# VUmcCGP/wisecondor

Hardware: AMD Instinct MI355X
Metric: newref bin-pair distances/sec (higher is better)
Workload: dtype f64; 1 GPU; cfg2: newref 100 samples x 250 kb bins (11087 masked bins, refsize 100); parallelism=newref sharded by single rank, symmetric tiles, 1 rank(s), world_size=1

## Files before the change

### wisecondor_amd/csrc/newref.hip

```cpp
#include <cstring>
#include "ctx.h"

#include <algorithm>
#include <stdlib.h>

namespace {

constexpr int TB = 128;
constexpr int BK = 32;
constexpr int LDA = 36;
constexpr int LDT = 68;
constexpr int ROLE_ROWS = 1;
constexpr int ROLE_COLS = 2;
constexpr int MAX_SAMPLE_COLS = 4096;
constexpr int LIST_CAP = 1024;
constexpr int K_MAX = 1024;
constexpr int GL_ROW = 16;
constexpr int GL_STAGE = 2 * TB * GL_ROW;
#define WC_ADMIT_ALL FLT_MAX
constexpr double SENTINEL_DISTANCE = 1e10;

typedef float f32x16 __attribute__((ext_vector_type(16)));
typedef float f32x4 __attribute__((ext_vector_type(4)));
typedef _Float16 f16x8 __attribute__((ext_vector_type(8)));
// ... 772 lines not shown
            for (int o = 32; o > 0; o >>= 1) my = fmax(my, __shfl_xor(my, o));
            if (lane == 0) red[tid >> 6] = my;
            wc_sync();
            U = red[0];
            for (int q = 1; q < NT / 64; ++q) U = fmax(U, red[q]);
            if (!(U == U) || (!admit_all && !(U <= (double)thr_f))) fallback = true;
        }
        {
            const float bad = *a.bad_norm;
            if (bad < INFINITY) {
                const double ni = sqrt(fmax((double)a.norm_lo[row] + (double)nhi_f, 0.0));
                if (!((sqrt(fmax(U, 0.0)) + ni) * (1.0 + 1e-3) < (double)bad * (1.0 - 1e-3))) fallback = true;
            }
        }
        if (!fallback) {
            for (int t0 = 0; t0 < n; t0 += NT) {
                int t = t0 + tid;
                bool keep = false;
                int j = 0;
                if (t < n) {
                    j = (int)(uint32_t)ent[t];
                    keep = (double)wc::f32_from_ordered((uint32_t)(ent[t] >> 32)) <= U;
                }
                unsigned long long m = __ballot(keep);
                int base = 0;
                if (lane == 0 && m) base = atomicAdd(&s_tmp[2], __popcll(m));
                base = __shfl(base, 0);
                int at = base + __popcll(m & ((1ull << lane) - 1ull));
                if (keep && at < RMAX) cj[at] = j;
            }
            wc_sync();
            R = s_tmp[2];
            if (R > RMAX) fallback = true;
        }
    }
    if (fallback) {
        if (tid == 0) {
            int at = atomicAdd(a.fb_count, 1);
            a.fb_rows[at] = (int)row;
            a.row_stat[row] = -1;
        }
        return;
    }

    {
        constexpr bool seq = SEQ;
        const int l8 = tid & 7, r0 = tid >> 3;
        for (int b0 = 0; b0 < R; b0 += CB) {
            const int nb = (R - b0) < CB ? (R - b0) : CB;
            unsigned int src[NP];
            f64x2 pre[NP];
            auto fetch = [&](unsigned int so) {
                if ((int64_t)so + ST_CH <= a.S) {
#pragma unroll
                    for (int p = 0; p < NP; ++p) pre[p] = *(const f64x2_u *)&a.X[src[p] + so];
                } else {
                    const int64_t s0 = (int64_t)so + 2 * l8;
#pragma unroll
                    for (int p = 0; p < NP; ++p) {
                        pre[p].x = s0 < a.S ? a.X[src[p] + so] : 0.0;
                        pre[p].y = s0 + 1 < a.S ? a.X[src[p] + so + 1] : 0.0;
                    }
                }
            };
#pragma unroll
            for (int p = 0; p < NP; ++p) {
                int rr = r0 + RP * p;
                src[p] = (unsigned int)cj[b0 + (rr < nb ? rr : 0)] * (unsigned int)a.S + 2u * (unsigned int)l8;
            }
            fetch(0u);
            double acc = 0.0;
            double r[8] = {0, 0, 0, 0, 0, 0, 0, 0};
            double vs[10] = {0, 0, 0, 0, 0, 0, 0, 0, 0, 0};
            int sp = 0, leaf = 0;
            bool in_tail = false;
            int2 lf = seq ? make_int2(0, 0) : a.pw_prog[0];
            for (int64_t c0 = 0; c0 < a.S; c0 += ST_CH) {
                wc_sync();
                {
                    f64x2 x2;
                    if (c0 + ST_CH <= a.S && a.xs_in_lds) {
                        x2 = *(const f64x2 *)&xi[c0 + 2 * l8];
                    } else {
                        const int64_t s0 = c0 + 2 * l8;
                        x2.x = s0 < a.S ? xi[s0] : 0.0;
                        x2.y = s0 + 1 < a.S ? xi[s0 + 1] : 0.0;
                    }
#pragma unroll
                    for (int p = 0; p < NP; ++p) {
                        const double d0 = pre[p].x - x2.x, d1 = pre[p].y - x2.y;
                        f64x2 sq2;
                        sq2.x = d0 * d0;
                        sq2.y = d1 * d1;
                        *(f64x2 *)&stage[(r0 + RP * p) * ST_LD + 2 * l8] = sq2;
                    }
                }
                wc_sync();
                if (c0 + ST_CH < a.S) fetch((unsigned int)(c0 + ST_CH));
                if (SEQ && tid < CB && c0 + ST_CH <= a.S && a.xs_in_lds) {
                    const double *sp_ = &stage[tid * ST_LD];
#pragma unroll
                    for (int e = 0; e < ST_CH; e += 2) {
                        const f64x2 v = *(const f64x2 *)(sp_ + e);
                        acc = acc + v.x;
                        acc = acc + v.y;
                    }
                } else if (tid < CB) {
                    const bool full = c0 + ST_CH <= a.S && a.xs_in_lds;
#pragma unroll
                    for (int g = 0; g < 2; ++g) {
                        const int64_t base = c0 + 8 * g;
                        if (base >= a.S) break;
                        const int cntg = (a.S - base) < 8 ? (int)(a.S - base) : 8;
                        double sq[8];
                        if (full) {
                            const double *sp_ = &stage[tid * ST_LD + 8 * g];
#pragma unroll
                            for (int e = 0; e < 8; e += 2) {
                                const f64x2 v = *(const f64x2 *)(sp_ + e);
                                sq[e] = v.x;
                                sq[e + 1] = v.y;
                            }
                        } else {
#pragma unroll
                            for (int e = 0; e < 8; ++e) sq[e] = (e < cntg) ? stage[tid * ST_LD + 8 * g + e] : 0.0;
                        }
                        if (seq || in_tail || cntg < 8) {
                            for (int e = 0; e < cntg; ++e) acc = acc + sq[e];
                        } else {
#pragma unroll
                            for (int e = 0; e < 8; ++e) r[e] = r[e] + sq[e];
                            if (base + 8 == (int64_t)(lf.x - (lf.x & 7))) {
                                double val = ((r[0] + r[1]) + (r[2] + r[3])) + ((r[4] + r[5]) + (r[6] + r[7]));
#pragma unroll
                                for (int e = 0; e < 8; ++e) r[e] = 0.0;
                                if (lf.x & 7) {
                                    acc = val;
                                    in_tail = true;
                                } else {
                                    wc::stack_set(vs, sp++, val);
                                    for (int q = 0; q < lf.y; ++q) {
                                        double right = wc::stack_get(vs, --sp), left = wc::stack_get(vs, sp - 1);
                                        wc::stack_set(vs, sp - 1, left + right);
                                    }
                                    ++leaf;
                                    if (leaf < a.pw_leaves) lf = a.pw_prog[leaf];
                                }
                            }
                        }
                    }
                }
            }
            if (!seq) {
                if (in_tail) {
                    wc::stack_set(vs, sp++, acc);
                    for (int q = 0; q < lf.y; ++q) {
                        double right = wc::stack_get(vs, --sp), left = wc::stack_get(vs, sp - 1);
                        wc::stack_set(vs, sp - 1, left + right);
                    }
                }
                acc = vs[0];
            }
            if (tid < nb) {
                bool ok = acc < SENTINEL_DISTANCE;
                dk[b0 + tid] = ok ? wc::f64_ordered(acc) : ~0ull;
                jv[b0 + tid] = ok ? cj[b0 + tid] : 0x40000000 + b0 + tid;
            }
        }
    }
    const int64_t cs = a.chrom_off[ch], ce = a.chrom_off[ch + 1];
    const int64_t orow = row - a.row_begin;
    wc_sync();
    {
        if (tid == 0 && (R & 1)) { dk[R] = ~0ull; jv[R] = 0x7FFFFFFF; }
        wc_sync();
        for (int t = tid; t < R; t += NT) {
            const unsigned long long mine = dk[t];
            const int myj = jv[t];
            int rank = 0;
            for (int u = 0; u < R; u += 2) {
                const u64x2 kk = *(const u64x2 *)&dk[u];
                const int2 jj = *(const int2 *)&jv[u];
                rank += (kk.x < mine) | ((kk.x == mine) & (jj.x < myj));
                rank += (kk.y < mine) | ((kk.y == mine) & (jj.y < myj));
            }
            if (rank < a.k) {
                int32_t oi = -1;
                double od = SENTINEL_DISTANCE;
                if (mine != ~0ull) {
                    oi = (int32_t)(myj < cs ? myj : myj - (ce - cs));
                    od = wc::f64_from_ordered(mine);
                }
                a.idx_out[orow * a.k + rank] = oi;
                a.dist_out[orow * a.k + rank] = od;
            }
        }
        for (int t = R + tid; t < a.k; t += NT) {
            a.idx_out[orow * a.k + t] = -1;
            a.dist_out[orow * a.k + t] = SENTINEL_DISTANCE;
        }
    }
    if (tid == 0) a.row_stat[row] = R;
}

constexpr int PS_MAX = 512;

struct PickArgs {
    FinishArgs f;
    int *pairs;
    int ps;
};

template <int NE, bool LEAN>
__device__ inline int pick_row(const PickArgs &p, int64_t row, int lane, int n, bool admit_all, float thr_f,
                               float nhi_f, const unsigned long long (&spec)[8]) {
    const FinishArgs &a = p.f;
    const unsigned long long *lst = a.list + row * a.cap;
    unsigned long long ent[LEAN ? 1 : NE];
    float nh[LEAN ? 1 : NE];
    uint32_t key[LEAN ? NE : 1];
    if constexpr (LEAN) {
#pragma unroll
        for (int e = 0; e < NE; ++e) {
            const int t = e * 64 + lane;
            key[e] = t < n ? (uint32_t)((e < 8 ? spec[e] : lst[t]) >> 32) : 0xFFFFFFFFu;
        }
    } else {
#pragma unroll
        for (int e = 0; e < NE; ++e) {
            const int t = e * 64 + lane;
            ent[e] = t < n ? (e < 8 ? spec[e] : lst[t]) : ~0ull;
        }
#pragma unroll
        for (int e = 0; e < NE; ++e) {
            const int t = e * 64 + lane;
            nh[e] = t < n ? a.norm_hi[(int)(uint32_t)ent[e]] : 0.f;
        }
    }
    auto KU = [&](int e) -> uint32_t { if constexpr (LEAN) return key[e]; else return (uint32_t)(ent[e] >> 32); };
    auto IDX = [&](int e) -> uint32_t { if constexpr (LEAN) return (uint32_t)lst[e * 64 + lane]; else return (uint32_t)ent[e]; };
    double U = INFINITY;
    if (n < a.k) {
        if (!admit_all) return -1;
    } else {
        uint32_t kmin = 0xFFFFFFFFu, kmax = 0u;
#pragma unroll
        for (int e = 0; e < NE; ++e)
            if (e * 64 + lane < n) {
                const uint32_t ku = KU(e);
                kmin = ku < kmin ? ku : kmin;
                kmax = ku > kmax ? ku : kmax;
            }
        for (int o = 32; o > 0; o >>= 1) {
            const uint32_t a2 = (uint32_t)__shfl_xor((int)kmin, o), b2 = (uint32_t)__shfl_xor((int)kmax, o);
            kmin = a2 < kmin ? a2 : kmin;
            kmax = b2 > kmax ? b2 : kmax;
        }
        long long lo = (long long)kmin - 1, hi = (long long)kmax;
        uint32_t res = kmax;
        while (hi - lo > 4096) {
            const uint32_t trial = (uint32_t)(lo + ((hi - lo) >> 1));
            int c = 0;
#pragma unroll
            for (int e = 0; e < NE; ++e) c += __popcll(__ballot(KU(e) <= trial));
            if (c >= a.k) { hi = (long long)trial; res = trial; if (c == a.k) break; }
            else lo = (long long)trial;
        }
        const double nhi = (double)nhi_f;
        double my = -INFINITY;
#pragma unroll
        for (int e = 0; e < NE; ++e) {
            const uint32_t ku = KU(e);
            if (e * 64 + lane < n && ku <= res) {
                float slack;
                if constexpr (LEAN) slack = a.norm_hi[(int)IDX(e)]; else slack = nh[e];
                const double ub = (double)wc::f32_from_ordered(ku) + (nhi + (double)slack) + 1e-36;
                my = fmax(my, ub);
            }
        }
        for (int o = 32; o > 0; o >>= 1) my = fmax(my, __shfl_xor(my, o));
        U = my;
        if (!(U == U) || (!admit_all && !(U <= (double)thr_f))) return -1;
    }
    {
        const float bad = *a.bad_norm;
        if (bad < INFINITY) {
            const double ni = sqrt(fmax((double)a.norm_lo[row] + (double)nhi_f, 0.0));
            if (!((sqrt(fmax(U, 0.0)) + ni) * (1.0 + 1e-3) < (double)bad * (1.0 - 1e-3))) return -1;
        }
    }
    int base = 0;
    int *out = p.pairs + row * RMAX;
#pragma unroll
    for (int e = 0; e < NE; ++e) {
        const bool keep = e * 64 + lane < n && (double)wc::f32_from_ordered(KU(e)) <= U;
        const unsigned long long m = __ballot(keep);
        const int at = base + __popcll(m & ((1ull << lane) - 1ull));
        if (keep && at < RMAX) out[at] = (int)IDX(e);
        base += __popcll(m);
    }
    return base;
}

__global__ __launch_bounds__(256, 7) void k_pick(PickArgs p) {
    const FinishArgs &a = p.f;
    const int lane = threadIdx.x & 63;
    const int64_t row = a.row_begin + (int64_t)blockIdx.x * 4 + (threadIdx.x >> 6);
    if (row >= a.row_end) return;
    unsigned long long spec[8];
#pragma unroll
    for (int e = 0; e < 8; ++e) spec[e] = a.list[row * a.cap + e * 64 + lane];
    const int c = a.cnt[row];
    const float thr_f = a.thr[row];
    const float nhi_f = a.norm_hi[row];
    const int ch = a.chrom_of_row[row];
    const bool admit_all = (thr_f == WC_ADMIT_ALL);
    const bool exact = c > a.cap || ((a.lone_mask >> ch) & 1ull);
    int R = -1;
    if (!exact) R = c <= 512 ? pick_row<8, false>(p, row, lane, c, admit_all, thr_f, nhi_f, spec)
                             : pick_row<LIST_CAP / 64, true>(p, row, lane, c, admit_all, thr_f, nhi_f, spec);
    if (lane != 0) return;
    if (R < 0 || R > RMAX) {
        const int at = atomicAdd(a.fb_count, 1);
        a.fb_rows[at] = (int)row;
        a.row_stat[row] = -1;
        return;
    }
    a.row_stat[row] = R;
}

__device__ inline void vs_set(double (&v)[8], int i, double x) {
    switch (i) {
        case 0: v[0] = x; break; case 1: v[1] = x; break; case 2: v[2] = x; break; case 3: v[3] = x; break;
        case 4: v[4] = x; break; case 5: v[5] = x; break; case 6: v[6] = x; break; default: v[7] = x; break;
    }
}
__device__ inline double vs_get(const double (&v)[8], int i) {
    switch (i) {
        case 0: return v[0]; case 1: return v[1]; case 2: return v[2]; case 3: return v[3];
        case 4: return v[4]; case 5: return v[5]; case 6: return v[6]; default: return v[7];
    }
}

template <bool SEQ>
struct RowSum {
    double acc;
    double r[8];
    double vs[8];
    int sp, leaf;
    bool in_tail;
    int2 lf;
    __device__ inline void init(const FinishArgs &a) {
        acc = 0.0;
#pragma unroll
        for (int e = 0; e < 8; ++e) r[e] = 0.0;
#pragma unroll
        for (int e = 0; e < 8; ++e) vs[e] = 0.0;
        sp = 0; leaf = 0; in_tail = false;
        lf = SEQ ? make_int2(0, 0) : a.pw_prog[0];
    }
    __device__ inline void chunk_regs(const FinishArgs &a, const double (&v)[ST_CH], int64_t c0, bool full) {
        if (SEQ) {
#pragma unroll
            for (int e = 0; e < ST_CH; ++e) acc = acc + v[e];
            return;
        }
#pragma unroll
        for (int g = 0; g < 2; ++g) {
            const int64_t base = c0 + 8 * g;
            if (base >= a.S) break;
            const int cntg = full ? 8 : ((a.S - base) < 8 ? (int)(a.S - base) : 8);
            if (in_tail || cntg < 8) {
#pragma unroll
                for (int e = 0; e < 8; ++e)
                    if (e < cntg) acc = acc + v[8 * g + e];
            } else {
#pragma unroll
                for (int e = 0; e < 8; ++e) r[e] = r[e] + v[8 * g + e];
                leaf_end(a, base);
            }
        }
    }
    __device__ inline void group_regs(const FinishArgs &a, const double (&v)[8], int64_t base, int cntg) {
        if (in_tail || cntg < 8) {
#pragma unroll
            for (int e = 0; e < 8; ++e)
                if (e < cntg) acc = acc + v[e];
        } else {
#pragma unroll
            for (int e = 0; e < 8; ++e) r[e] = r[e] + v[e];
            leaf_end(a, base);
        }
    }
    __device__ inline void leaf_end(const FinishArgs &a, int64_t base) {
        if (base + 8 == (int64_t)(lf.x - (lf.x & 7))) {
            const double val = ((r[0] + r[1]) + (r[2] + r[3])) + ((r[4] + r[5]) + (r[6] + r[7]));
#pragma unroll
            for (int e = 0; e < 8; ++e) r[e] = 0.0;
            if (lf.x & 7) {
                acc = val;
                in_tail = true;
            } else {
                vs_set(vs, sp++, val);
                for (int q = 0; q < lf.y; ++q) {
                    const double right = vs_get(vs, --sp), left = vs_get(vs, sp - 1);
                    vs_set(vs, sp - 1, left + right);
                }
                ++leaf;
                if (leaf < a.pw_leaves) lf = a.pw_prog[leaf];
            }
        }
    }
    __device__ inline double result() {
        if (SEQ) return acc;
        if (in_tail) {
            vs_set(vs, sp++, acc);
            for (int q = 0; q < lf.y; ++q) {
                const double right = vs_get(vs, --sp), left = vs_get(vs, sp - 1);
                vs_set(vs, sp - 1, left + right);
            }
        }
        return vs[0];
    }
};

__device__ inline void wave_lds_fence() {
    __builtin_amdgcn_fence(__ATOMIC_RELEASE, "wavefront");
    __builtin_amdgcn_wave_barrier();
    __builtin_amdgcn_fence(__ATOMIC_ACQUIRE, "wavefront");
}

constexpr int SLAB_DOUBLES = 64 * ST_CH;
template <bool SEQ, bool GLDS>
__global__ __launch_bounds__(PS_MAX, (SEQ && !GLDS) ? 4 : (SEQ ? 5 : 3)) void k_rescore(PickArgs p, const double *__restrict__ Xp, int Sp) {
    const FinishArgs &a = p.f;
    extern __shared__ __attribute__((aligned(16))) double rs_dyn[];
    const int tid = threadIdx.x, lane = tid & 63, w = __builtin_amdgcn_readfirstlane(tid >> 6);
    const int64_t row = a.row_begin + blockIdx.x;
    const int cj_first = p.pairs[row * RMAX + tid];
    const int R = a.row_stat[row];
    double *xs = rs_dyn;
    char *slab = reinterpret_cast<char *>(rs_dyn + Sp + w * SLAB_DOUBLES);
    {
        const double *xi = Xp + row * Sp;
        for (int s = tid; s < Sp; s += p.ps) xs[s] = xi[s];
    }
    if (R < 0) return;
    wc_sync();
    const int l8 = lane & 7, r0 = lane >> 3;
    constexpr int NP = 8;
    constexpr int TRIPS = RMAX / 128;
    auto swz = [](int r) { return ((r >> 1) & 3) | (((r >> 4) & 1) << 2); };
    int waddr[NP], raddr[NP];
#pragma unroll
    for (int q = 0; q < NP; ++q) {
        const int rw = r0 + 8 * q;
        waddr[q] = rw * 128 + ((l8 ^ swz(rw)) << 4);
        raddr[q] = lane * 128 + ((q ^ swz(lane)) << 4);
    }
    unsigned long long my_d[TRIPS];
    int my_j[TRIPS];
    int trip = 0;
    const int nchunk = Sp / ST_CH;
    const char *base = reinterpret_cast<const char *>(Xp);
    for (int b0 = w * 64; b0 < R; b0 += p.ps, ++trip) {
        const int nb = R - b0 < 64 ? R - b0 : 64;
        const int *cjp = p.pairs + row * RMAX + b0;
        int cj = trip == 0 ? cj_first : cjp[lane < nb ? lane : 0];
        if (trip == 0) cj = __shfl(cj, lane < nb ? lane : 0);
        unsigned int src[NP];
        RowSum<SEQ> sum;
        sum.init(a);
        if constexpr (GLDS) {
            const int l4 = lane & 3, rq = lane >> 2;
#pragma unroll
            for (int j = 0; j < 4; ++j) {
                const int rw = 16 * j + rq;
                src[j] = ((unsigned int)__shfl(cj, rw) * (unsigned int)Sp + 2u * (unsigned int)(l4 ^ ((rw >> 2) & 3))) * 8u;
            }
            int rd[4];
#pragma unroll
            for (int q = 0; q < 4; ++q) rd[q] = lane * 64 + ((q ^ ((lane >> 2) & 3)) << 4);
            auto dma = [&](int c, int half) {
                const char *cb = base + (size_t)c * (ST_CH * 8) + half * 64;
                char *dst = slab + half * 4096;
#pragma unroll
                for (int j = 0; j < 4; ++j)
                    __builtin_amdgcn_global_load_lds((glb_void_t *)(cb + src[j]), (lds_void_t *)(dst + j * 1024), 16, 0, 0);
            };
            dma(0, 0);
            dma(0, 1);
            for (int c = 0; c < nchunk; ++c) {
                __builtin_amdgcn_s_waitcnt(0x0070);
                __builtin_amdgcn_wave_barrier();
                f64x2 t[8];
#pragma unroll
                for (int q = 0; q < 4; ++q) t[q] = *(const f64x2 *)(slab + rd[q]);
#pragma unroll
                for (int q = 0; q < 4; ++q) t[4 + q] = *(const f64x2 *)(slab + 4096 + rd[q]);
                __builtin_amdgcn_s_waitcnt(0xC07F);
                __builtin_amdgcn_wave_barrier();
                if (c + 1 < nchunk) { dma(c + 1, 0); dma(c + 1, 1); }
                double v[ST_CH];
#pragma unroll
                for (int q = 0; q < NP; ++q) {
                    const f64x2 x2 = *(const f64x2 *)&xs[c * ST_CH + 2 * q];
                    const double d0 = t[q].x - x2.x, d1 = t[q].y - x2.y;
                    v[2 * q] = d0 * d0;
                    v[2 * q + 1] = d1 * d1;
                }
                sum.chunk_regs(a, v, (int64_t)c * ST_CH, (c + 1) * ST_CH <= a.S);
            }
        } else {
#pragma unroll
        for (int q = 0; q < NP; ++q)
            src[q] = ((unsigned int)__shfl(cj, r0 + 8 * q) * (unsigned int)Sp + 2u * (unsigned int)l8) * 8u;
        f64x2 pre[NP];
#pragma unroll
        for (int q = 0; q < NP; ++q) pre[q] = *(const f64x2 *)(base + src[q]);
        for (int c = 0; c < nchunk; ++c) {
            const f64x2 x2 = *(const f64x2 *)&xs[c * ST_CH + 2 * l8];
            wave_lds_fence();
#pragma unroll
            for (int q = 0; q < NP; ++q) {
                const double d0 = pre[q].x - x2.x, d1 = pre[q].y - x2.y;
                f64x2 sq2;
                sq2.x = d0 * d0;
                sq2.y = d1 * d1;
                *(f64x2 *)(slab + waddr[q]) = sq2;
            }
            wave_lds_fence();
            if (c + 1 < nchunk) {
                const char *cb = base + (size_t)(c + 1) * (ST_CH * 8);
#pragma unroll
                for (int q = 0; q < NP; ++q) pre[q] = *(const f64x2 *)(cb + src[q]);
            }
            double v[ST_CH];
#pragma unroll
            for (int q = 0; q < NP; ++q) {
                const f64x2 t2 = *(const f64x2 *)(slab + raddr[q]);
                v[2 * q] = t2.x;
                v[2 * q + 1] = t2.y;
            }
            sum.chunk_regs(a, v, (int64_t)c * ST_CH, (c + 1) * ST_CH <= a.S);
        }
        }
        const double d = sum.result();
        const bool ok = lane < nb && d < SENTINEL_DISTANCE;
        const unsigned long long dd = ok ? wc::f64_ordered(d) : ~0ull;
        const int jj = ok ? cj : 0x40000000 + b0 + lane;
#pragma unroll
        for (int t = 0; t < TRIPS; ++t)
            if (t == trip) { my_d[t] = dd; my_j[t] = jj; }
    }
    wc_sync();
    unsigned long long *dk = reinterpret_cast<unsigned long long *>(rs_dyn + Sp);
    unsigned long long *sd = dk + RMAX + 2;
    int *jv = reinterpret_cast<int *>(sd + RMAX);
    int *sj = jv + RMAX + 2;
    {
        int t2 = 0;
        for (int b0 = w * 64; b0 < R; b0 += p.ps, ++t2) {
#pragma unroll
            for (int t = 0; t < TRIPS; ++t)
                if (t == t2 && b0 + lane < R) { dk[b0 + lane] = my_d[t]; jv[b0 + lane] = my_j[t]; }
        }
    }
    if (tid == 0 && (R & 1)) dk[R] = ~0ull;
    for (int t = tid; t < R; t += p.ps) sj[t] = -1;
    wc_sync();
    for (int t = tid; t < R; t += p.ps) {
        const unsigned long long mine = dk[t];
        int rank = 0;
        for (int u = 0; u < R; u += 2) {
            const u64x2 kk = *(const u64x2 *)&dk[u];
            rank += kk.x < mine;
            rank += kk.y < mine;
        }
        sd[rank] = mine;
        sj[rank] = jv[t];
    }
    wc_sync();
    int hole = 0;
    for (int t = tid; t < R; t += p.ps) hole |= sj[t] == -1;
    if (wc_sync_or(hole)) {
        for (int t = tid; t < R; t += p.ps) {
            const unsigned long long mine = dk[t];
            const int myj = jv[t];
            int rank = 0;
            for (int u = 0; u < R; ++u) rank += (dk[u] < mine) | ((dk[u] == mine) & (jv[u] < myj));
            sd[rank] = mine;
            sj[rank] = myj;
        }
        wc_sync();
    }
    const int ch = a.chrom_of_row[row];
    const int64_t cs = a.chrom_off[ch], ce = a.chrom_off[ch + 1];
    const int64_t orow = row - a.row_begin;
    for (int t = tid; t < a.k; t += p.ps) {
        int32_t oi = -1;
        double od = SENTINEL_DISTANCE;
        if (t < R && sd[t] != ~0ull) {
            const int myj = sj[t];
            oi = (int32_t)(myj < cs ? myj : myj - (ce - cs));
            od = wc::f64_from_ordered(sd[t]);
        }
        a.idx_out[orow * a.k + t] = oi;
        a.dist_out[orow * a.k + t] = od;
    }
}

template <bool SEQ>
__device__ inline void fb_fill_order(const FinishArgs &a, int64_t row, const double *xi, int64_t j0, int64_t j1,
                                     unsigned long long *__restrict__ sc, int tid) {
    const int ch = a.chrom_of_row[row];
    const int64_t cs = a.chrom_off[ch], ce = a.chrom_off[ch + 1];
    for (int64_t base = j0; base < j1; base += 256) {
        const int64_t j = base + tid;
        const bool in = j < j1;
        const double *xj = a.X + (in ? j : row) * a.S;
        RowSum<SEQ> sum;
        sum.init(a);
        for (int64_t c0 = 0; c0 < a.S; c0 += ST_CH) {
            double v[ST_CH];
#pragma unroll
            for (int e = 0; e < ST_CH; ++e) {
                const double d = c0 + e < a.S ? xj[c0 + e] - xi[c0 + e] : 0.0;
                v[e] = d * d;
            }
            sum.chunk_regs(a, v, c0, c0 + ST_CH <= a.S);
        }
// ... 495 lines not shown
    if (st.pw_for != n_samples) {
        std::vector<int2> prog;
        build_pairwise_leaves((int)n_samples, 0, prog);
        if ((rc = st.pw_prog.reserve(sizeof(int2) * prog.size()))) return rc;
        WC_HIP(hipMemcpyAsync(st.pw_prog.p, prog.data(), sizeof(int2) * prog.size(), hipMemcpyHostToDevice, stream));
        WC_HIP(hipStreamSynchronize(stream));
        st.pw_leaves = (int)prog.size();
        st.pw_for = n_samples;
    }
    std::vector<int64_t> skey = {n_bins, M};
    if (skey != st.sample_key) {
        int64_t real = std::min<int64_t>(M, n_bins);
        std::vector<int> perm(n_bins);
        for (int64_t i = 0; i < n_bins; ++i) perm[i] = (int)i;
        uint64_t s = 0x9E3779B97F4A7C15ull;
        for (int64_t i = 0; i < real; ++i) {
            s = s * 6364136223846793005ull + 1442695040888963407ull;
            int64_t pick = i + (int64_t)((s >> 33) % (uint64_t)(n_bins - i));
            std::swap(perm[i], perm[pick]);
        }
        std::sort(perm.begin(), perm.begin() + real);
        std::vector<int> slot((size_t)n_bins, -1);
        for (int64_t i = 0; i < real; ++i) slot[perm[i]] = (int)i;
        WC_HIP(hipMemcpyAsync(st.sample_rows.p, perm.data(), sizeof(int) * real, hipMemcpyHostToDevice, stream));
        WC_HIP(hipMemcpyAsync(st.sample_slot.p, slot.data(), sizeof(int) * n_bins, hipMemcpyHostToDevice, stream));
        WC_HIP(hipStreamSynchronize(stream));
        st.sample_key = skey;
        st.tiles0_key.clear();
        st.tiles1_key.clear();
    }

    double *mean2 = st.col_mean.as<double>();
    {
        int64_t n_rows = std::min<int64_t>(n_bins, 128);
        int64_t row_step = n_bins / n_rows;
        hipLaunchKernelGGL(k_col_centre, dim3((unsigned)((n_samples + 63) / 64)), dim3(1024), 0, stream, corrected,
                           n_bins, n_samples, n_rows, row_step, mean2, st.m2.as<int>() + 1);
    }

    hipLaunchKernelGGL(k_convert, dim3((unsigned)(st.bins_pad / 8)), dim3(256), 0, stream, corrected, n_bins,
                       n_samples, st.bins_pad, (const double *)mean2, (double)st.beta, st.tau,
                       st.chrom_off_dev.as<int64_t>(), n_chrom, st.a16.as<unsigned short>(),
                       st.k_pad16, st.norm_lo.as<float>(), st.norm_hi.as<float>(), st.chrom_of_row.as<int>(),
                       st.chrom_range.as<int2>(), (const int *)st.sample_slot.as<int>(),
                       st.s16.as<unsigned short>(), st.s_norm_lo.as<float>(), st.s_chrom.as<int>(),
                       st.s_range.as<int2>(), st.thr.as<float>(), st.cnt.as<int>(), st.stats.as<int>(),
                       st.x64_pad ? st.x64.as<double>() : (double *)nullptr, st.s_pad, st.m2.as<float>(),
                       st.m2.as<int>() + 1, st.fb_count.as<int>(), 4);
    st.fb_dirty = false;
    if (M > n_bins)
        hipLaunchKernelGGL(k_pad_samples, dim3((unsigned)(M - n_bins)), dim3(256), 0, stream, st.k_pad16, n_bins,
                           st.s16.as<unsigned short>(), st.s_norm_lo.as<float>(), st.s_chrom.as<int>(),
                           st.s_range.as<int2>());
    WC_HIP(hipGetLastError());
    st.prepared = true;
    return WC_OK;
}

int wc_newref_thresholds_dev(wc_ctx *ctx, void *stream_, int64_t row_begin, int64_t row_end) {
    WC_CHECK(ctx && ctx->nr.prepared, WC_E_ARG, "newref: prepare has not run");
    NewrefState &st = ctx->nr;
    WC_CHECK(row_begin >= 0 && row_begin <= row_end && row_end <= st.n_bins, WC_E_ARG, "newref: bad row range");
    if (row_begin == row_end || st.exact_only) return WC_OK;
    hipStream_t stream = (hipStream_t)stream_;
    const int ib = (int)(row_begin / TB), ie = (int)((row_end + TB - 1) / TB);
    const int mb = (int)(st.n_sample_cols / TB);
    std::vector<int64_t> key = {st.bins_pad, st.n_sample_cols, ib, ie};
    if (key != st.tiles0_key) {
        std::vector<int4> tiles;
        tiles.reserve((size_t)(ie - ib) * mb);
        for (int I = ib; I < ie; ++I)
            for (int J = 0; J < mb; ++J) tiles.push_back(make_int4(I, J, 0, 0));
        int rc;
        if ((rc = st.tiles0.reserve(sizeof(int4) * tiles.size()))) return rc;
        WC_HIP(hipMemcpyAsync(st.tiles0.p, tiles.data(), sizeof(int4) * tiles.size(), hipMemcpyHostToDevice, stream));
        WC_HIP(hipStreamSynchronize(stream));
        st.tiles0_key = key;
        st.tiles0_n = (int64_t)tiles.size();
    }
    {
        const int ntiles = (int)st.tiles0_n;
        unsigned grid = (unsigned)(((ntiles + 7) / 8) * 8);
        hipLaunchKernelGGL(k_gram_thr16, dim3(grid), dim3(256), 0, stream,
                           (const unsigned short *)st.a16.as<unsigned short>(),
                           (const unsigned short *)st.s16.as<unsigned short>(), st.k_pad16, (int)(st.k_pad16 / 64),
                           (const float *)st.norm_lo.as<float>(), (const float *)st.s_norm_lo.as<float>(),
                           (const int2 *)st.s_range.as<int2>(), (const int4 *)st.tiles0.as<int4>(), ntiles,
                           st.keys1.as<unsigned int>(), st.n_sample_cols, (const float *)st.m2.as<float>());
    }
    unsigned sg = (unsigned)((row_end - row_begin + 3) / 4);
    {
        const unsigned int *kp = st.keys1.as<unsigned int>();
        const int2 *cr = st.chrom_range.as<int2>();
        const int per_lane = (int)(st.n_sample_cols / 64);
#define WC_SELECT(NV)                                                                                          \
    hipLaunchKernelGGL(k_select_thr<NV>, dim3(sg), dim3(256), 0, stream, kp, st.n_sample_cols,                \
                       (int)st.n_sample_cols, cr, st.n_bins, row_begin, row_end, (int)st.expect, (int)st.cap, \
                       st.thr.as<float>())
        if (per_lane <= 16) WC_SELECT(16);
        else if (per_lane <= 32) WC_SELECT(32);
        else WC_SELECT(64);
#undef WC_SELECT
    }
    WC_HIP(hipGetLastError());
    return WC_OK;
}

int64_t wc_newref_list_capacity(wc_ctx *ctx) { return ctx ? ctx->nr.cap : 0; }

int wc_newref_get_thresholds_dev(wc_ctx *ctx, void *stream, int64_t row_begin, int64_t row_end, float *out) {
    WC_CHECK(ctx && ctx->nr.prepared && out, WC_E_ARG, "newref: bad argument");
    WC_CHECK(row_begin >= 0 && row_begin <= row_end && row_end <= ctx->nr.n_bins, WC_E_ARG, "newref: bad row range");
    if (row_end > row_begin)
        WC_HIP(hipMemcpyAsync(out, ctx->nr.thr.as<float>() + row_begin, sizeof(float) * (row_end - row_begin),
                              hipMemcpyDeviceToDevice, (hipStream_t)stream));
    return WC_OK;
}

int wc_newref_get_bounds_dev(wc_ctx *ctx, void *stream, int64_t row_begin, int64_t row_end, float *lo_out,
                             float *slack_out) {
    WC_CHECK(ctx && ctx->nr.prepared && lo_out && slack_out, WC_E_ARG, "newref: bad argument");
    WC_CHECK(row_begin >= 0 && row_begin <= row_end && row_end <= ctx->nr.n_bins, WC_E_ARG, "newref: bad row range");
    if (row_end > row_begin) {
        WC_HIP(hipMemcpyAsync(lo_out, ctx->nr.norm_lo.as<float>() + row_begin, sizeof(float) * (row_end - row_begin),
                              hipMemcpyDeviceToDevice, (hipStream_t)stream));
        WC_HIP(hipMemcpyAsync(slack_out, ctx->nr.norm_hi.as<float>() + row_begin, sizeof(float) * (row_end - row_begin),
                              hipMemcpyDeviceToDevice, (hipStream_t)stream));
    }
    return WC_OK;
}

int wc_newref_set_thresholds_dev(wc_ctx *ctx, void *stream, int64_t row_begin, int64_t row_end, const float *in) {
    WC_CHECK(ctx && ctx->nr.prepared && in, WC_E_ARG, "newref: bad argument");
    WC_CHECK(row_begin >= 0 && row_begin <= row_end && row_end <= ctx->nr.n_bins, WC_E_ARG, "newref: bad row range");
    if (row_end > row_begin)
        WC_HIP(hipMemcpyAsync(ctx->nr.thr.as<float>() + row_begin, in, sizeof(float) * (row_end - row_begin),
                              hipMemcpyDeviceToDevice, (hipStream_t)stream));
    return WC_OK;
}

int wc_newref_export_lists_dev(wc_ctx *ctx, void *stream, int64_t row_begin, int64_t row_end, int64_t dst_cap,
                               int32_t *dst_cnt, uint64_t *dst_list) {
    WC_CHECK(ctx && ctx->nr.prepared && dst_cnt && dst_list && dst_cap > 0, WC_E_ARG, "newref: bad argument");
    WC_CHECK(row_begin >= 0 && row_begin <= row_end && row_end <= ctx->nr.n_bins, WC_E_ARG, "newref: bad row range");
    if (row_end == row_begin) return WC_OK;
    NewrefState &st = ctx->nr;
    hipLaunchKernelGGL(k_export_lists, dim3((unsigned)(row_end - row_begin)), dim3(64), 0, (hipStream_t)stream,
                       (const int *)st.cnt.as<int>(), (const unsigned long long *)st.list.as<unsigned long long>(),
                       (int)st.cap, row_begin, (int)dst_cap, dst_cnt, (unsigned long long *)dst_list);
    WC_HIP(hipGetLastError());
    return WC_OK;
}

int wc_newref_import_lists_dev(wc_ctx *ctx, void *stream, int64_t row_begin, int64_t row_end, int64_t src_cap,
                               const int32_t *src_cnt, const uint64_t *src_list) {
    WC_CHECK(ctx && ctx->nr.prepared && src_cnt && src_list && src_cap > 0, WC_E_ARG, "newref: bad argument");
    WC_CHECK(row_begin >= 0 && row_begin <= row_end && row_end <= ctx->nr.n_bins, WC_E_ARG, "newref: bad row range");
    if (row_end == row_begin) return WC_OK;
    NewrefState &st = ctx->nr;
    hipLaunchKernelGGL(k_import_lists, dim3((unsigned)(row_end - row_begin)), dim3(64), 0, (hipStream_t)stream,
                       st.cnt.as<int>(), st.list.as<unsigned long long>(), (int)st.cap, row_begin, (int)src_cap,
                       src_cnt, (const unsigned long long *)src_list);
    WC_HIP(hipGetLastError());
    return WC_OK;
}

int wc_newref_collect_dev(wc_ctx *ctx, void *stream_, int64_t row_begin, int64_t row_end, int tile_rank,
                          int tile_ranks) {
    WC_CHECK(ctx && ctx->nr.prepared, WC_E_ARG, "newref: prepare has not run");
    NewrefState &st = ctx->nr;
    WC_CHECK(row_begin >= 0 && row_begin <= row_end && row_end <= st.n_bins, WC_E_ARG, "newref: bad row range");
    WC_CHECK(tile_ranks >= 1 && tile_rank >= 0 && tile_rank < tile_ranks, WC_E_ARG, "newref: bad tile rank");
    if (row_begin == row_end || st.exact_only) return WC_OK;
    hipStream_t stream = (hipStream_t)stream_;
    std::vector<int64_t> key = {st.n_bins, row_begin, row_end, tile_rank, tile_ranks};
    for (int c = 0; c <= st.n_chrom; ++c) key.push_back(st.chrom_off[c]);
    if (key != st.tiles1_key) {
        std::vector<int4> tiles;
        build_tiles(st, row_begin, row_end, tile_rank, tile_ranks, tiles);
        int rc;
        if ((rc = st.tiles.reserve(sizeof(int4) * std::max<size_t>(tiles.size(), 1)))) return rc;
        if (!tiles.empty()) {
            WC_HIP(hipMemcpyAsync(st.tiles.p, tiles.data(), sizeof(int4) * tiles.size(), hipMemcpyHostToDevice, stream));
            WC_HIP(hipStreamSynchronize(stream));
        }
        st.tiles1_key = key;
        st.tiles1_n = (int64_t)tiles.size();
    }
    ctx->last_stats[2] = st.tiles1_n;
    ctx->last_stats[3] = st.n_sample_cols;
    if (st.tiles1_n == 0) return WC_OK;
    GramArgs g{};
    g.P = g.Q = st.a16.as<float>();
    g.ld = st.k_pad16 / 2;
    g.m2 = st.m2.as<float>();
    g.nslab32 = (int)((st.n_samples + 31) / 32);
    g.last_steps32 = (int)(((st.n_samples - (int64_t)(g.nslab32 - 1) * 32) + 15) / 16);
    g.nbP = g.nbQ = st.norm_lo.as<float>();
    g.range = st.chrom_range.as<int2>();
    g.tiles = st.tiles.as<int4>();
    g.ntiles = (int)st.tiles1_n;
    g.thr = st.thr.as<float>();
    g.cnt = st.cnt.as<int>();
    g.list = st.list.as<unsigned long long>();
    g.cap = (int)st.cap;
    const unsigned grid = (unsigned)(((g.ntiles + 7) / 8) * 8);
    hipLaunchKernelGGL(k_gram_glds, dim3(grid), dim3(256), 0, stream, g);
    WC_HIP(hipGetLastError());
    return WC_OK;
}

static void finish_args(NewrefState &st, int64_t row_begin, int64_t row_end, int32_t *idx_out, double *dist_out,
                        FinishArgs &a) {
    a.X = st.corrected;
    a.B = st.n_bins;
    a.S = st.n_samples;
    a.norm_lo = st.norm_lo.as<float>();
    a.norm_hi = st.norm_hi.as<float>();
    a.thr = st.thr.as<float>();
    a.cnt = st.cnt.as<int>();
    a.list = st.list.as<unsigned long long>();
    a.cap = (int)st.cap;
    a.k = st.k;
    a.beta = (double)st.beta;
    a.chrom_of_row = st.chrom_of_row.as<int>();
    a.chrom_off = st.chrom_off_dev.as<int64_t>();
    a.row_begin = row_begin;
    a.row_end = row_end;
    a.idx_out = idx_out;
    a.dist_out = dist_out;
    a.fb_rows = st.fb_rows.as<int>();
    a.fb_count = st.fb_count.as<int>();
    a.bad_norm = st.m2.as<float>() + 1;
    a.row_stat = st.stats.as<int>();
    a.sum_order = st.sum_order;
    a.lone_mask = 0ull;
    if (st.sum_order == WC_SUM_SEQUENTIAL)
        for (int c = 0; c < st.n_chrom; ++c)
            if (st.chrom_off[c] <= 1 && st.n_bins - st.chrom_off[c + 1] <= 1) a.lone_mask |= 1ull << c;
    a.xs_in_lds = st.n_samples <= 2048;
    a.pw_prog = st.pw_prog.as<int2>();
    a.pw_leaves = st.pw_leaves;
}

static int launch_exact(NewrefState &st, hipStream_t stream, const FinishArgs &a, int64_t n_host) {
    int rc;
    const int cap = n_host < 0 ? EX_DEV_CAP : EX_CAP;
    if ((rc = st.fb_scratch.reserve(sizeof(uint64_t) * (n_host < 0 ? 2 : 1) * cap * st.bins_pad))) return rc;
    const bool seq = st.sum_order == WC_SUM_SEQUENTIAL || st.n_samples < 8;
    const int edge = seq ? 64 : 32;
    const unsigned ctiles = (unsigned)((st.n_bins + edge - 1) / edge);
    unsigned long long *scratch = st.fb_scratch.as<unsigned long long>();
    const int *rows = st.fb_rows.as<int>();
    if (n_host < 0) {
        const int rgroups = 4;
        int *sync = st.fb_count.as<int>() + 1;
        constexpr int EXD_TILE_WGS = 192, EXD_SEL_WGS = 64;
        const int n_tile = (int)std::min<int64_t>((int64_t)ctiles * rgroups, EXD_TILE_WGS);
        const unsigned grid = (unsigned)(n_tile + EXD_SEL_WGS);
        if (seq) hipLaunchKernelGGL((k_exact_dev<true>), dim3(grid), dim3(256), 0, stream, a, rows,
                                    (const int *)st.fb_count.as<int>(), sync, scratch, st.bins_pad, cap, (int)ctiles, rgroups, EXD_SEL_WGS);
        else hipLaunchKernelGGL((k_exact_dev<false>), dim3(grid), dim3(256), 0, stream, a, rows,
                                (const int *)st.fb_count.as<int>(), sync, scratch, st.bins_pad, cap, (int)ctiles, rgroups, EXD_SEL_WGS);
        return WC_OK;
    }
    for (int64_t first = 0; first < n_host; first += cap) {
        const int64_t nf = std::min<int64_t>(cap, n_host - first);
        const unsigned rgroups = (unsigned)((nf + edge - 1) / edge);
        if (seq) hipLaunchKernelGGL((k_exact_tile<true>), dim3(ctiles, rgroups), dim3(256), 0, stream, a, rows,
                                    (const int *)nullptr, (int)n_host, (int)first, scratch, st.bins_pad, cap);
        else hipLaunchKernelGGL((k_exact_tile<false>), dim3(ctiles, rgroups), dim3(256), 0, stream, a, rows,
                                (const int *)nullptr, (int)n_host, (int)first, scratch, st.bins_pad, cap);
        hipLaunchKernelGGL(k_exact_select, dim3((unsigned)nf), dim3(256), 0, stream, a, rows, (int)n_host, (int)first,
                           scratch, st.bins_pad, cap);
    }
    return WC_OK;
}

static int newref_finish_part(wc_ctx *ctx, void *stream_, int64_t row_begin, int64_t row_end, int32_t *idx_out,
                              double *dist_out, int which) {
    WC_CHECK(ctx && ctx->nr.prepared, WC_E_ARG, "newref: prepare has not run");
    NewrefState &st = ctx->nr;
    WC_CHECK(row_begin >= 0 && row_begin <= row_end && row_end <= st.n_bins, WC_E_ARG, "newref: bad row range");
    WC_CHECK(idx_out && dist_out, WC_E_ARG, "newref: NULL output");
    if (row_begin == row_end) return WC_OK;
    hipStream_t stream = (hipStream_t)stream_;
    int rc;
    if (which & 5) {
        if (st.fb_dirty) WC_HIP(hipMemsetAsync(st.fb_count.p, 0, sizeof(int) * 4, stream));
        st.fb_dirty = true;
    }
    FinishArgs a{};
    finish_args(st, row_begin, row_end, idx_out, dist_out, a);
    const int ps = (int)std::max<int64_t>(128, std::min<int64_t>(PS_MAX, round_up(st.k + 28, 64)));
    const bool pair_engine = st.x64_pad && !st.exact_only;
    if ((which & 12) && !pair_engine) which = (which & ~12) | ((which & 4) ? 1 : 0);
    const bool seq = st.sum_order == WC_SUM_SEQUENTIAL || st.n_samples < 8;
    const unsigned rows = (unsigned)(row_end - row_begin);
    if ((which & 1) && st.exact_only) {
        hipLaunchKernelGGL(k_all_exact, dim3((rows + 255) / 256), dim3(256), 0, stream, a);
    } else if ((which & 13) && pair_engine) {
        if ((rc = st.pairs.reserve(sizeof(int) * st.bins_pad * RMAX))) return rc;
        PickArgs p{a, st.pairs.as<int>(), ps};
        if (which & 5) hipLaunchKernelGGL(k_pick, dim3((rows + 3) / 4), dim3(256), 0, stream, p);
        const size_t slabs = sizeof(double) * (size_t)(ps / 64) * SLAB_DOUBLES;
        const size_t order = (sizeof(unsigned long long) + sizeof(int)) * (2 * RMAX + 4);
        const size_t dyn = sizeof(double) * st.s_pad + std::max(slabs, order);
        if (!(which & 9)) {
        } else if (seq) hipLaunchKernelGGL((k_rescore<true, false>), dim3(rows), dim3(ps), dyn, stream, p,
                                           (const double *)st.x64.as<double>(), (int)st.s_pad);
        else hipLaunchKernelGGL((k_rescore<false, true>), dim3(rows), dim3(ps), dyn, stream, p,
                                (const double *)st.x64.as<double>(), (int)st.s_pad);
    } else if (which & 1) {
        const size_t dyn = a.xs_in_lds ? sizeof(double) * st.n_samples : 0;
        if (seq) hipLaunchKernelGGL((k_finish<true, 128>), dim3(rows), dim3(128), dyn, stream, a);
        else hipLaunchKernelGGL((k_finish<false, 128>), dim3(rows), dim3(128), dyn, stream, a);
    }
    if (which & 2) {
        if (st.exact_only) rc = launch_exact(st, stream, a, (int64_t)rows);
        else rc = launch_exact(st, stream, a, -1);
        if (rc) return rc;
    }
    WC_HIP(hipGetLastError());
    return WC_OK;
}

int wc_newref_exact_dev(wc_ctx *ctx, void *stream_, int64_t row_begin, int64_t row_end, int32_t *idx_out,
                        double *dist_out) {
    WC_CHECK(ctx && ctx->nr.prepared, WC_E_ARG, "newref: prepare has not run");
    NewrefState &st = ctx->nr;
    WC_CHECK(row_begin >= 0 && row_begin <= row_end && row_end <= st.n_bins, WC_E_ARG, "newref: bad row range");
    WC_CHECK(idx_out && dist_out, WC_E_ARG, "newref: NULL output");
    if (row_begin == row_end) return WC_OK;
    hipStream_t stream = (hipStream_t)stream_;
    FinishArgs a{};
    finish_args(st, row_begin, row_end, idx_out, dist_out, a);
    const unsigned rows = (unsigned)(row_end - row_begin);
    hipLaunchKernelGGL(k_all_exact, dim3((rows + 255) / 256), dim3(256), 0, stream, a);
    st.fb_dirty = true;
    const int rc = launch_exact(st, stream, a, (int64_t)rows);
    if (rc) return rc;
    WC_HIP(hipGetLastError());
    return WC_OK;
}

int wc_newref_finish_dev(wc_ctx *ctx, void *stream, int64_t row_begin, int64_t row_end, int32_t *idx_out,
                         double *dist_out) {
    return newref_finish_part(ctx, stream, row_begin, row_end, idx_out, dist_out, 3);
}

int wc_newref_rescore_dev(wc_ctx *ctx, void *stream, int64_t row_begin, int64_t row_end, int32_t *idx_out,
                          double *dist_out) {
    return newref_finish_part(ctx, stream, row_begin, row_end, idx_out, dist_out, 1);
}

int wc_newref_fallback_dev(wc_ctx *ctx, void *stream, int64_t row_begin, int64_t row_end, int32_t *idx_out,
                           double *dist_out) {
    return newref_finish_part(ctx, stream, row_begin, row_end, idx_out, dist_out, 2);
}

int wc_newref_pick_dev(wc_ctx *ctx, void *stream, int64_t row_begin, int64_t row_end, int32_t *idx_out,
                       double *dist_out) {
    return newref_finish_part(ctx, stream, row_begin, row_end, idx_out, dist_out, 4);
}

int wc_newref_rescore_pairs_dev(wc_ctx *ctx, void *stream, int64_t row_begin, int64_t row_end, int32_t *idx_out,
                                double *dist_out) {
    return newref_finish_part(ctx, stream, row_begin, row_end, idx_out, dist_out, 8);
}

__global__ void k_noop(int *p) {
    if (p && threadIdx.x == 9999) *p = 0;
}

int wc_launch_floor_us(wc_ctx *ctx, void *stream_, int n, int reps, double *out) {
    WC_CHECK(ctx && out && n > 0 && reps > 0, WC_E_ARG, "launch floor: bad argument");
    WC_HIP(hipSetDevice(ctx->device));
    hipStream_t stream = (hipStream_t)stream_;
    hipEvent_t e0, e1;
    WC_HIP(hipEventCreate(&e0));
    WC_HIP(hipEventCreate(&e1));
    for (int i = 0; i < n; ++i) hipLaunchKernelGGL(k_noop, dim3(1), dim3(64), 0, stream, (int *)nullptr);
    WC_HIP(hipStreamSynchronize(stream));
    WC_HIP(hipEventRecord(e0, stream));
    for (int r = 0; r < reps; ++r)
        for (int i = 0; i < n; ++i) hipLaunchKernelGGL(k_noop, dim3(1), dim3(64), 0, stream, (int *)nullptr);
    WC_HIP(hipEventRecord(e1, stream));
    WC_HIP(hipEventSynchronize(e1));
    float ms = 0.f;
    WC_HIP(hipEventElapsedTime(&ms, e0, e1));
    (void)hipEventDestroy(e0);
    (void)hipEventDestroy(e1);
    out[0] = 1e3 * (double)ms / (double)reps;
    return WC_OK;
}

static int newref_pass(wc_ctx *ctx, void *stream, const double *corrected, int64_t n_bins, int64_t n_samples,
                       const int64_t *chrom_bins_host, int n_chrom, int k, int sum_order, int64_t row_begin,
                       int64_t row_end, int32_t *idx_out, double *dist_out) {
    int rc = wc_newref_prepare_dev(ctx, stream, corrected, n_bins, n_samples, chrom_bins_host, n_chrom, k,
                                   sum_order);
    if (rc) return rc;
    if ((rc = wc_newref_thresholds_dev(ctx, stream, row_begin, row_end))) return rc;
    if ((rc = wc_newref_collect_dev(ctx, stream, row_begin, row_end, 0, 1))) return rc;
    return wc_newref_finish_dev(ctx, stream, row_begin, row_end, idx_out, dist_out);
}

int wc_get_reference_dev(wc_ctx *ctx, void *stream_, const double *corrected, int64_t n_bins, int64_t n_samples,
                         const int64_t *chrom_bins_host, int n_chrom, int k, int sum_order,
                         int64_t row_begin, int64_t row_end, int32_t *idx_out, double *dist_out) {
    WC_CHECK(ctx && corrected && chrom_bins_host, WC_E_ARG, "newref: NULL argument");
    return newref_pass(ctx, stream_, corrected, n_bins, n_samples, chrom_bins_host, n_chrom, k, sum_order,
                       row_begin, row_end, idx_out, dist_out);
}

int wc_get_reference(wc_ctx *ctx, const double *corrected, int64_t n_bins, int64_t n_samples,
                     const int64_t *chrom_bins, int n_chrom, int k, int sum_order, int64_t row_begin,
                     int64_t row_end, int32_t *idx_out, double *dist_out) {
    WC_CHECK(ctx && corrected && idx_out && dist_out, WC_E_ARG, "getReference: NULL argument");
    WC_CHECK(row_begin >= 0 && row_begin <= row_end && row_end <= n_bins, WC_E_ARG, "getReference: bad row range");
    WC_HIP(hipSetDevice(ctx->device));
    int64_t rows = row_end - row_begin;
    int rc;
    if ((rc = ctx->tmp_a.reserve(sizeof(double) * n_bins * n_samples))) return rc;
    if ((rc = ctx->tmp_b.reserve(sizeof(int32_t) * std::max<int64_t>(rows, 1) * k))) return rc;
    if ((rc = ctx->tmp_c.reserve(sizeof(double) * std::max<int64_t>(rows, 1) * k))) return rc;
    WC_HIP(hipMemcpy(ctx->tmp_a.p, corrected, sizeof(double) * n_bins * n_samples, hipMemcpyHostToDevice));
    rc = wc_get_reference_dev(ctx, nullptr, ctx->tmp_a.as<double>(), n_bins, n_samples, chrom_bins, n_chrom, k,
                              sum_order, row_begin, row_end, ctx->tmp_b.as<int32_t>(), ctx->tmp_c.as<double>());
    if (rc) return rc;
    WC_HIP(hipDeviceSynchronize());
    if (rows > 0) {
        WC_HIP(hipMemcpy(idx_out, ctx->tmp_b.p, sizeof(int32_t) * rows * k, hipMemcpyDeviceToHost));
        WC_HIP(hipMemcpy(dist_out, ctx->tmp_c.p, sizeof(double) * rows * k, hipMemcpyDeviceToHost));
    }
    return WC_OK;
}

int wc_newref_stats(wc_ctx *ctx, int64_t out[8]) {
    WC_CHECK(ctx && out, WC_E_ARG, "stats: NULL argument");
    for (int i = 0; i < 8; ++i) out[i] = 0;
    NewrefState &st = ctx->nr;
    if (st.stats.p && st.prepared) {
        WC_HIP(hipSetDevice(ctx->device));
        WC_HIP(hipDeviceSynchronize());
        std::vector<int> rows(st.n_bins);
        WC_HIP(hipMemcpy(rows.data(), st.stats.p, sizeof(int) * st.n_bins, hipMemcpyDeviceToHost));
        for (int64_t r = 0; r < st.n_bins; ++r) {
            if (rows[r] >= 0) { out[0] += 1; out[4] += rows[r]; }
            else if (rows[r] == -1) out[1] += 1;
        }
    }
    out[2] = ctx->last_stats[2];
    out[3] = ctx->last_stats[3];
    return WC_OK;
}

}
```

Measured before the change: 624.5 billion bin-pair distances/s.

## Process two rows per wavefront in k_pick using half-wave reductions

```diff
diff --git a/wisecondor_amd/csrc/newref.hip b/wisecondor_amd/csrc/newref.hip
--- a/wisecondor_amd/csrc/newref.hip
+++ b/wisecondor_amd/csrc/newref.hip
@@ -1098,24 +1098,103 @@
     return base;
 }
 
-__global__ __launch_bounds__(256, 7) void k_pick(PickArgs p) {
+template <int O>
+__device__ inline int half_xor(int v) { return __builtin_amdgcn_ds_swizzle(v, 0x1F | (O << 10)); }
+template <int O>
+__device__ inline void half_minmax(uint32_t &kmin, uint32_t &kmax) {
+    const uint32_t a2 = (uint32_t)half_xor<O>((int)kmin), b2 = (uint32_t)half_xor<O>((int)kmax);
+    kmin = a2 < kmin ? a2 : kmin;
+    kmax = b2 > kmax ? b2 : kmax;
+}
+template <int O>
+__device__ inline void half_fmax(double &v) {
+    const long long b = __double_as_longlong(v);
+    const uint32_t lo = (uint32_t)half_xor<O>((int)(uint32_t)b), hi = (uint32_t)half_xor<O>((int)(uint32_t)(b >> 32));
+    v = fmax(v, __longlong_as_double((long long)(((unsigned long long)hi << 32) | lo)));
+}
+
+__device__ inline int pick_row2(const PickArgs &p, int64_t row0, int hl, bool upper, bool live, int n, bool admit_all,
+                                float thr_f, float nhi_f, const unsigned long long (&ent)[16]) {
     const FinishArgs &a = p.f;
-    const int lane = threadIdx.x & 63;
-    const int64_t row = a.row_begin + (int64_t)blockIdx.x * 4 + (threadIdx.x >> 6);
-    if (row >= a.row_end) return;
-    unsigned long long spec[8];
-#pragma unroll
-    for (int e = 0; e < 8; ++e) spec[e] = a.list[row * a.cap + e * 64 + lane];
-    const int c = a.cnt[row];
-    const float thr_f = a.thr[row];
-    const float nhi_f = a.norm_hi[row];
-    const int ch = a.chrom_of_row[row];
-    const bool admit_all = (thr_f == WC_ADMIT_ALL);
-    const bool exact = c > a.cap || ((a.lone_mask >> ch) & 1ull);
-    int R = -1;
-    if (!exact) R = c <= 512 ? pick_row<8, false>(p, row, lane, c, admit_all, thr_f, nhi_f, spec)
-                             : pick_row<LIST_CAP / 64, true>(p, row, lane, c, admit_all, thr_f, nhi_f, spec);
-    if (lane != 0) return;
+    const int up = live && upper ? 1 : 0;
+    constexpr int NE = 16;
+    auto KU = [&](int e) -> uint32_t { return (uint32_t)(ent[e] >> 32); };
+    auto HALF = [&](unsigned long long m) -> uint32_t { return upper ? (uint32_t)(m >> 32) : (uint32_t)m; };
+    bool ok = live && (n >= a.k || admit_all);
+    const bool bis = live && n >= a.k;
+    double U = INFINITY;
+    {
+        uint32_t kmin = 0xFFFFFFFFu, kmax = 0u;
+#pragma unroll
+        for (int e = 0; e < NE; ++e)
+            if (e * 32 + hl < n) {
+                const uint32_t ku = KU(e);
+                kmin = ku < kmin ? ku : kmin;
+                kmax = ku > kmax ? ku : kmax;
+            }
+        half_minmax<16>(kmin, kmax); half_minmax<8>(kmin, kmax); half_minmax<4>(kmin, kmax);
+        half_minmax<2>(kmin, kmax); half_minmax<1>(kmin, kmax);
+        uint32_t lo1 = bis ? kmin : 0u, hi = bis ? kmax : 0u;
+        uint32_t res = kmax;
+        bool run = hi - lo1 >= 4096u;
+        while (__ballot(run) != 0ull) {
+            const uint32_t d = hi - lo1;
+            const uint32_t trial = lo1 - 1u + (d >> 1) + (d & 1u);
+            int c = 0;
+#pragma unroll
+            for (int e = 0; e < NE; ++e) c += __popc(HALF(__ballot(KU(e) <= trial)));
+            if (run) {
+                if (c >= a.k) { hi = trial; res = trial; run = c != a.k; }
+                else lo1 = trial + 1u;
+                run = run && hi - lo1 >= 4096u;
+            }
+        }
+        const double nhi = (double)nhi_f;
+        double my = -INFINITY;
+#pragma unroll
+        for (int g = 0; g < NE; g += 8) {
+            float slack[8];
+#pragma unroll
+            for (int e = g; e < g + 8; ++e) {
+                slack[e - g] = 0.f;
+                if (bis && KU(e) <= res && KU(e) != 0xFFFFFFFFu) slack[e - g] = a.norm_hi[(int)(uint32_t)ent[e]];
+            }
+#pragma unroll
+            for (int e = g; e < g + 8; ++e) {
+                const uint32_t ku = KU(e);
+                if (ku <= res) {
+                    const double ub = (double)wc::f32_from_ordered(ku) + (nhi + (double)slack[e - g]) + 1e-36;
+                    my = fmax(my, ub);
+                }
+            }
+        }
+        half_fmax<16>(my); half_fmax<8>(my); half_fmax<4>(my); half_fmax<2>(my); half_fmax<1>(my);
+        if (bis) {
+            U = my;
+            if (!(U == U) || (!admit_all && !(U <= (double)thr_f))) ok = false;
+        }
+    }
+    {
+        const float bad = *a.bad_norm;
+        if (bad < INFINITY) {
+            const double ni = sqrt(fmax((double)a.norm_lo[row0 + up] + (double)nhi_f, 0.0));
+            if (!((sqrt(fmax(U, 0.0)) + ni) * (1.0 + 1e-3) < (double)bad * (1.0 - 1e-3))) ok = false;
+        }
+    }
+    int base = 0;
+    int *out = p.pairs + row0 * RMAX + up * RMAX;
+#pragma unroll
+    for (int e = 0; e < NE; ++e) {
+        const bool keep = ok && (double)wc::f32_from_ordered(KU(e)) <= U;
+        const uint32_t m = HALF(__ballot(keep));
+        const int at = base + __popc(m & ((1u << hl) - 1u));
+        if (keep && at < RMAX) out[at] = (int)(uint32_t)ent[e];
+        base += __popc(m);
+    }
+    return ok ? base : -1;
+}
+
+__device__ inline void pick_publish(const FinishArgs &a, int64_t row, int R) {
     if (R < 0 || R > RMAX) {
         const int at = atomicAdd(a.fb_count, 1);
         a.fb_rows[at] = (int)row;
@@ -1123,6 +1202,55 @@
         return;
     }
     a.row_stat[row] = R;
+}
+
+__global__ __launch_bounds__(256, 6) void k_pick(PickArgs p) {
+    const FinishArgs &a = p.f;
+    const int lane = threadIdx.x & 63, hl = lane & 31;
+    const bool upper = lane >= 32;
+    const int64_t row0 = a.row_begin + ((int64_t)blockIdx.x * 4 + __builtin_amdgcn_readfirstlane(threadIdx.x >> 6)) * 2;
+    if (row0 >= a.row_end) return;
+    const bool has_row = row0 + (upper ? 1 : 0) < a.row_end;
+    const int64_t row = has_row && upper ? row0 + 1 : row0;
+    unsigned long long ent[16];
+#pragma unroll
+    for (int e = 0; e < 16; ++e) ent[e] = a.list[row * a.cap + e * 32 + hl];
+    const int c = a.cnt[row];
+    const float thr_f = a.thr[row];
+    const float nhi_f = a.norm_hi[row];
+    int ch = a.chrom_of_row[row];
+    asm volatile("" : "+v"(ch));
+    const bool admit_all = (thr_f == WC_ADMIT_ALL);
+    const bool exact = c > a.cap || ((a.lone_mask >> ch) & 1ull);
+    const bool whole = __ballot(has_row && (exact || c > 512)) != 0ull;
+    const bool live = has_row && !whole;
+    const int n = live ? c : 0;
+#pragma unroll
+    for (int e = 0; e < 16; ++e)
+        if (e * 32 + hl >= n) ent[e] = ~0ull;
+    const int R2 = pick_row2(p, row0, hl, upper, live, n, admit_all, thr_f, nhi_f, ent);
+    if (!whole) {
+        if (hl == 0 && has_row) pick_publish(a, row0 + (upper ? 1 : 0), R2);
+        return;
+    }
+    int wl = lane;
+    asm volatile("" : "+v"(wl));
+    auto whole_wave = [&](int64_t r) {
+        const int c1 = a.cnt[r];
+        const float thr1 = a.thr[r], nhi1 = a.norm_hi[r];
+        const bool exact1 = c1 > a.cap || ((a.lone_mask >> a.chrom_of_row[r]) & 1ull);
+        int R = -1;
+        if (!exact1) {
+            unsigned long long spec[8];
+#pragma unroll
+            for (int e = 0; e < 8; ++e) spec[e] = a.list[r * a.cap + e * 64 + wl];
+            R = c1 <= 512 ? pick_row<8, false>(p, r, wl, c1, thr1 == WC_ADMIT_ALL, thr1, nhi1, spec)
+                          : pick_row<LIST_CAP / 64, true>(p, r, wl, c1, thr1 == WC_ADMIT_ALL, thr1, nhi1, spec);
+        }
+        if (wl == 0) pick_publish(a, r, R);
+    };
+    whole_wave(row0);
+    if (row0 + 1 < a.row_end) whole_wave(row0 + 1);
 }
 
 __device__ inline void vs_set(double (&v)[8], int i, double x) {
@@ -2224,7 +2352,7 @@
     } else if ((which & 13) && pair_engine) {
         if ((rc = st.pairs.reserve(sizeof(int) * st.bins_pad * RMAX))) return rc;
         PickArgs p{a, st.pairs.as<int>(), ps};
-        if (which & 5) hipLaunchKernelGGL(k_pick, dim3((rows + 3) / 4), dim3(256), 0, stream, p);
+        if (which & 5) hipLaunchKernelGGL(k_pick, dim3((rows + 7) / 8), dim3(256), 0, stream, p);
         const size_t slabs = sizeof(double) * (size_t)(ps / 64) * SLAB_DOUBLES;
         const size_t order = (sizeof(unsigned long long) + sizeof(int)) * (2 * RMAX + 4);
         const size_t dyn = sizeof(double) * st.s_pad + std::max(slabs, order);
```

Result: slower. 614.7 billion bin-pair distances/s (-1.6%).
